# mingdeyu/DGP

Measured on AMD Instinct MI355X. Metric: SI iterations/sec (train) + predict pts/sec, 2-layer DGP n=2000 d=5, higher is better.
Workload: dtype f64; 1 GPU; configs[1]: 2-layer DGP, d=5 in / 1 out, n=2000, Matern-2.5, 5+1 GP nodes, train(ess_burn=10): one step = imputer.sample() + the M-step = one iteration of dgp.train (dgp.py:1364-1412); the same rate over a train(N=100) call is in `sustained`

## Files before the change

### dgp_amd/_lib.py

```python
import ctypes as C
import os

_HERE = os.path.dirname(os.path.abspath(__file__))
LIB_PATH = os.environ.get('DGPAMD_LIB') or os.path.join(_HERE, 'libdgp_amd.so')

OK, NOT_PD, BAD_ARG, HIP_ERROR = 0, 1, 2, 3
SEXP, MATERN25 = 0, 1
MAXD, MAXB = 64, 64
KIND = {'sexp': SEXP, 'matern2.5': MATERN25}

if not os.path.exists(LIB_PATH):
    raise ImportError(
        'dgp_amd: %s not found -- build it with `python -c "import __graft_entry__ as g; g.build()"` '
        '(or `make -C dgp_amd/csrc`).  dgp_amd has no CPU fallback.' % LIB_PATH)

lib = C.CDLL(LIB_PATH)

_p = C.c_void_p
_i = C.c_int
_l = C.c_int64
_d = C.c_double
_z = C.c_size_t

class Node(C.Structure):
# ... 21 lines not shown
    'dgpamd_gemv': (_i, [_p, _l, _l, _p, _l, _p, _p]),
    'dgpamd_fetch': (_i, [_p, _p, _p, _z]),
    'dgpamd_fetch2': (_i, [_p, _p, _z, _p, _z, _p]),
    'dgpamd_set_reduce_hook': (_i, [_p, _p, _p]),
    'dgpamd_post': (_i, [_p, _p, _z, _i]),
    'dgpamd_collect': (_i, [_p, _i, _p, _z]),
    'dgpamd_set_graphs': (_i, [_p, _i]),
    'dgpamd_tuning_get': (_i, [_p, C.c_char_p, _p]),
    'dgpamd_set_linkgp_direct': (_i, [_p, _i]),
    'dgpamd_set_potrf_mode': (_i, [_p, _i]),
    'dgpamd_debug_trace': (_i, [_p, _p]),
    'dgpamd_debug_tasklog': (_i, [_p, _p, C.c_longlong]),
    'dgpamd_debug_mega_table': (_i, [_p, _l, _i, _i, _p, _l]),
    'dgpamd_prof_enable': (_i, [_p, _i]),
    'dgpamd_prof_event_overhead_us': (_i, [_p, C.POINTER(_d)]),
    'dgpamd_prof_collect': (_i, [_p, C.POINTER(_l), C.POINTER(_d), C.POINTER(_d)]),
    'dgpamd_kmatrix': (_i, [_p, _i, _l, _p, _l, _l, _p, _i, _p, _i, _p, _i, _d, _p, _p, _l, _l, _i, _p, _l, _l, _i, _i]),
    'dgpamd_potrf_workspace': (_z, [_l, _i]),
    'dgpamd_potrf': (_i, [_p, _l, _p, _l, _i, _p, _p, _p]),
    'dgpamd_aug_quad': (_i, [_p, _l, _p, _l, _i, _i, _p]),
    'dgpamd_loglik_finish': (_i, [_p, _l, _p, _l, _i, _p, _d, _p]),
    'dgpamd_loglik': (_i, [_p, _i, _l, _p, _l, _l, _p, _i, _p, _i, _p, _i, _d, _p, _d, _p, _p, _l, _i, _p, _p, _p]),
    'dgpamd_trmv_lower': (_i, [_p, _l, _p, _l, _p, _p, _p, _i]),
    'dgpamd_lik_workspace': (_z, [_i]),
    'dgpamd_lik_loglik': (_i, [_p, _p, _l, _i, _p, _l, _i, _p, _p]),
    'dgpamd_ess_propose': (_i, [_p, _l, _i, _p, _p, _p, _i, _p]),
    'dgpamd_potri': (_i, [_p, _l, _p, _p, _i, _p]),
    'dgpamd_potri_batched': (_i, [_p, _l, _p, _p, _l, _i, _i, _p]),
    'dgpamd_grad_workspace': (_z, [_l, _i]),
    'dgpamd_grad_reduce': (_i, [_p, _i, _l, _p, _l, _p, _i, _p, _i, _p, _i, _d, _p, _i, _p, _p, _p]),
    'dgpamd_ess_update': (_i, [_p, _l, _i, _p, _p, _p, _d, _d, _p, _p, _i, _i, _i, _p, _p, _p, _p, _p, _p]),
    'dgpamd_ess_queue_scratch': (_z, []),
    'dgpamd_ess_queue': (_i, [_p, _l, _i, _p, _p, _i, _p, _p, _i, _p, _p, _p, _i, _i, _i, _i, _i, _p, _p, _p, _p, _p]),
    'dgpamd_ess_queue_vwork': (_z, [_l, _i, _i]),
    'dgpamd_ess_queue_note_info': (_i, [_p, _p, _p, _i]),
    'dgpamd_llik_batch': (_i, [_p, _l, _i, _p, _p, _p, _p, _l, _p, _p, _p, _p, _l]),
    'dgpamd_llik_batch_launch': (_i, [_p, _l, _i, _p, _p, _p, _p, _l, _p, _p, _p, _l]),
    'dgpamd_llik_batch_wait': (_i, [_p, _p]),
    'dgpamd_potrf_inv': (_i, [_p, _l, _p, _p, _p, _l, _i, _p, _p, _p]),
    'dgpamd_gp_workspace': (_z, [_l, _l]),
    'dgpamd_gp_predict': (_i, [_p, _i, _l, _l, _i, _p, _p, _p, _i, _p, _l, _p, _i, _d, _d, _p, _p, _p]),
    'dgpamd_joint_workspace': (_z, [_l, _l, _i, _i]),
    'dgpamd_joint_cov': (_i, [_p, _i, _l, _l, _i, _i, _i, _p, _l, _p, _i, _p, _l, _p, _l, _l, _p, _l, _p, _i, _d, _d, _p, _l,
                              _p, _p]),
    'dgpamd_mvn_paths': (_i, [_p, _l, _i, _i, _i, _p, _l, _p, _l, _p, _l, _p, _l]),
    'dgpamd_linkgp_workspace': (_z, [_l, _l, _i]),
# ... 55 lines not shown
```

### dgp_amd/csrc/chol.hip

```cpp
#include "common.hpp"
#include "tile.hpp"
#include "diagfac.hpp"

__device__ __forceinline__ void diag_logdet(DiagShared &sh, int ncol, int k, int b, int bad, double *logdet, int32_t *info) {
    const int tid = threadIdx.x;
    if (tid < 64) {
        const double pv = sh.piv[tid];
        double v = (tid < ncol && pv > 0.0) ? log(pv) : 0.0;
#pragma unroll
        for (int off = 32; off > 0; off >>= 1) v += __shfl_down(v, off, 64);
        if (tid == 0) {
            const double ld0 = k == 0 ? 0.0 : __hip_atomic_load(logdet + b, __ATOMIC_RELAXED, __HIP_MEMORY_SCOPE_AGENT);
            __hip_atomic_store(logdet + b, ld0 + v, __ATOMIC_RELAXED, __HIP_MEMORY_SCOPE_AGENT);
            int inf = k == 0 ? 0 : __hip_atomic_load(info + b, __ATOMIC_RELAXED, __HIP_MEMORY_SCOPE_AGENT);
            if (bad && inf == 0) inf = k * 64 + bad;
            __hip_atomic_store(info + b, inf, __ATOMIC_RELAXED, __HIP_MEMORY_SCOPE_AGENT);
        }
    }
}

enum { G_TRTRI1 = 2, G_TRTRI2 = 3, G_LAUUM = 4 };

struct GemmArgs {
    double *A;
// ... 1145 lines not shown
        int q = t / r, q2 = t % r;
        quad[(int64_t)b * r * r + t] = -A[(int64_t)b * stride_a + (n + q) * ld + n + q2];
    }
}

struct TrmvArgs {
    const double *L;
    int64_t ld, stride_a, n;
    const double *z;
    double *out;
    double sscale[DGPAMD_MAXB];
};
__global__ __launch_bounds__(256) void trmv_lower_kernel(TrmvArgs a) {
    const int b = blockIdx.y, wave = threadIdx.x >> 6, lane = threadIdx.x & 63;
    const int64_t i = (int64_t)blockIdx.x * 4 + wave;
    if (i >= a.n) return;
    const double *row = a.L + (int64_t)b * a.stride_a + i * a.ld;
    const double *z = a.z + (int64_t)b * a.n;
    double s = 0.0;
    for (int64_t j = lane; j <= i; j += 64) s = fma(row[j], z[j], s);
#pragma unroll
    for (int off = 32; off > 0; off >>= 1) s += __shfl_down(s, off, 64);
    if (lane == 0) a.out[(int64_t)b * a.n + i] = a.sscale[b] * s;
}

size_t potrf_ws_doubles(int64_t n, int batch) {
    int64_t nbk = padded_dim(n) / 64;
    return (size_t)batch * nbk * 4096 + 2 * DGPAMD_MAXB;
}

static size_t mega_sync_bytes(int64_t nbk, int batch);
static size_t mega_sync_offset(int64_t n, int batch) {
    const size_t b = potrf_ws_doubles(n, batch) * sizeof(double) + 3 * DGPAMD_MAXB * sizeof(int32_t);
    return (b + 127) / 128 * 128;
}
static size_t mega_piv_offset(int64_t n, int batch) {
    return mega_sync_offset(n, batch) + mega_sync_bytes(padded_dim(n) / 64, batch);
}
extern "C" size_t dgpamd_potrf_workspace(int64_t n, int batch) {
    return mega_piv_offset(n, batch) + (size_t)batch * padded_dim(n) * sizeof(double);
}

struct TaskTable {
    int4 *dev = nullptr;
    std::vector<int> offset, count, nhead, npanel;
    std::vector<double> tile_ops;
// ... 482 lines not shown

extern "C" int dgpamd_gemv(dgpamd_ctx *ctx, int64_t rows, int64_t cols, const double *A, int64_t ld, const double *x,
                           double *out) {
    if (!ctx) return DGPAMD_BAD_ARG;
    if (rows <= 0 || cols <= 0 || !A || !x || !out || ld < cols) BAD_ARG(ctx, "bad arguments");
    hipLaunchKernelGGL(gemv_kernel, dim3((unsigned)((rows + 3) / 4)), dim3(256), 0, ctx->stream, A, ld, rows, cols, x, out);
    LAUNCH_CHECK(ctx);
    return DGPAMD_OK;
}

extern "C" int dgpamd_trmv_lower(dgpamd_ctx *ctx, int64_t n, const double *L, int64_t stride_a, const double *scale_h,
                                 const double *z, double *out, int batch) {
    if (!ctx) return DGPAMD_BAD_ARG;
    if (n <= 0 || !L || !z || !out || !scale_h) BAD_ARG(ctx, "null pointer or n <= 0");
    if (batch <= 0 || batch > DGPAMD_MAXB) BAD_ARG(ctx, "need 1 <= batch <= DGPAMD_MAXB");
    TrmvArgs a;
    a.L = L; a.ld = padded_dim(n); a.stride_a = stride_a; a.n = n; a.z = z; a.out = out;
    for (int b = 0; b < batch; ++b) a.sscale[b] = sqrt(scale_h[b]);
    hipLaunchKernelGGL(trmv_lower_kernel, dim3((unsigned)((n + 3) / 4), batch), dim3(256), 0, ctx->stream, a);
    LAUNCH_CHECK(ctx);
    return DGPAMD_OK;
}

static int potri_launches(dgpamd_ctx *ctx, int64_t n, double *A, double *Ainv, int64_t stride_a, int r, int batch,
                          void *work);

extern "C" int dgpamd_potri_batched(dgpamd_ctx *ctx, int64_t n, double *A, double *Ainv, int64_t stride_a, int r,
                                    int batch, void *work) {
    if (!ctx) return DGPAMD_BAD_ARG;
    if (n <= 0 || !A || !Ainv || !work || r < 0) BAD_ARG(ctx, "null pointer or n <= 0");
    if (batch <= 0 || batch > DGPAMD_MAXB) BAD_ARG(ctx, "need 1 <= batch <= DGPAMD_MAXB");
    const int64_t Np = padded_dim(n);
    if (n + r > Np) BAD_ARG(ctx, "too many right-hand sides");
    if (batch > 1 && stride_a < Np * Np) BAD_ARG(ctx, "stride_a < Np*Np");
    const std::array<uint64_t, 10> key = {2, (uint64_t)n, (uint64_t)r, (uint64_t)A, (uint64_t)Ainv, (uint64_t)work,
                                          (uint64_t)batch, (uint64_t)stride_a, 0, 0};
    return graph_run(ctx, key, [&]() { return potri_launches(ctx, n, A, Ainv, stride_a, r, batch, work); });
}

extern "C" int dgpamd_potri(dgpamd_ctx *ctx, int64_t n, double *A, double *Ainv, int r, void *work) {
    return dgpamd_potri_batched(ctx, n, A, Ainv, 0, r, 1, work);
}

static int potri_launches(dgpamd_ctx *ctx, int64_t n, double *A, double *Ainv, int64_t stride_a, int r, int batch,
                          void *work) {
    const int64_t Np = padded_dim(n);
// ... 22 lines not shown
```

### dgp_amd/csrc/train.hip

```cpp
#include "common.hpp"
#include "wave.hpp"

#include <math.h>

struct ProposeArgs {
    const double *F, *NU;
    double *FP;
    int64_t count;
    double th[DGPAMD_MAXB];
};
__global__ __launch_bounds__(256) void ess_propose_kernel(ProposeArgs a) {
    const int b = blockIdx.y;
    const double c = cos(a.th[b]), s = sin(a.th[b]);
    for (int64_t i = (int64_t)blockIdx.x * 256 + threadIdx.x; i < a.count; i += (int64_t)gridDim.x * 256)
        a.FP[(int64_t)b * a.count + i] = a.F[i] * c + a.NU[i] * s;
}

extern "C" int dgpamd_ess_propose(dgpamd_ctx *ctx, int64_t n, int M, const double *F, const double *NU,
                                  const double *theta_h, int batch, double *FP) {
    if (!ctx) return DGPAMD_BAD_ARG;
    if (n <= 0 || M <= 0 || !F || !NU || !theta_h || !FP) BAD_ARG(ctx, "null pointer or empty block");
    if (batch <= 0 || batch > DGPAMD_MAXB) BAD_ARG(ctx, "need 1 <= batch <= DGPAMD_MAXB");
    ProposeArgs a;
    a.F = F; a.NU = NU; a.FP = FP; a.count = n * M;
// ... 636 lines not shown
            }
            if (llh[b] > log_y) {
                used += b;
                proposals += b + 1;
                theta = th[b]; lo = blo[b]; hi = bhi[b];
                HIP_TRY(ctx, hipMemcpyAsync(F, FP + (int64_t)b * n * M, sizeof(double) * n * M, hipMemcpyDeviceToDevice,
                                            ctx->stream));
                return finish(0, llh[b], 0);
            }
        }
        used += nb - 1;
        proposals += nb;
        theta = th[nb - 1]; lo = blo[nb - 1]; hi = bhi[nb - 1];
        pending = true;
    }
}

enum { ES_THETA = 0, ES_LO, ES_HI, ES_PENDING, ES_CURSOR, ES_STATUS, ES_INFO, ES_LL, ES_LOGY, ES_PROPOSALS, ES_BATCHES,
       ES_UPDATES, ES_NWORDS = DGPAMD_ESS_STATE };
struct EssScratch {
    double th[DGPAMD_MAXB], lo[DGPAMD_MAXB], hi[DGPAMD_MAXB], cs[DGPAMD_MAXB], sn[DGPAMD_MAXB], ll[DGPAMD_MAXB], logdet[DGPAMD_MAXB];
    int32_t info[DGPAMD_MAXB], infomax[DGPAMD_MAXB];
    int32_t nb, done, acc, halt;
    double likpart[DGPAMD_MAXB * 32];
};
#define ESS_TWO_PI 6.283185307179586

__device__ void ess_prepare(double *st, const double *u, int nuni, int B, EssScratch *sc);
__global__ void ess_begin_kernel(double *st, const double *u, const double *logu, int nuni, EssScratch *sc, int upd, int B, int resume) {
    if (threadIdx.x) return;
    if (resume && upd == 0) {
        sc->done = 0;
        sc->halt = 0;
        ess_prepare(st, u, nuni, B, sc);
        return;
    }
    if (upd > 0 && !sc->done && st[ES_STATUS] == 0.0) st[ES_STATUS] = 3.0;
    sc->acc = -1;
    sc->nb = 0;
    if (st[ES_STATUS] != 0.0) { sc->done = 1; sc->halt = 1; return; }
    int cur = (int)st[ES_CURSOR];
    if (cur + 2 > nuni) { st[ES_STATUS] = 4.0; sc->done = 1; sc->halt = 1; return; }
    st[ES_LOGY] = st[ES_LL] + logu[cur];
    const double theta = ESS_TWO_PI * u[cur + 1];
    st[ES_THETA] = theta; st[ES_LO] = theta - ESS_TWO_PI; st[ES_HI] = theta; st[ES_PENDING] = 0.0;
    st[ES_CURSOR] = cur + 2;
    sc->done = 0;
    sc->halt = 0;
    ess_prepare(st, u, nuni, B, sc);
}
__device__ void ess_prepare(double *st, const double *u, int nuni, int B, EssScratch *sc) {
    sc->acc = -1;
    sc->nb = 0;
    if (sc->done) return;
    int cur = (int)st[ES_CURSOR];
    double theta = st[ES_THETA], lo = st[ES_LO], hi = st[ES_HI];
    if (st[ES_PENDING] != 0.0) {
        if (cur >= nuni) { st[ES_STATUS] = 1.0; sc->done = 1; return; }
        if (theta < 0.0) lo = theta; else hi = theta;
        theta = __dadd_rn(lo, __dmul_rn(hi - lo, u[cur++]));
        st[ES_THETA] = theta; st[ES_LO] = lo; st[ES_HI] = hi; st[ES_PENDING] = 0.0; st[ES_CURSOR] = cur;
    }
    int nb = 1;
    sc->th[0] = theta; sc->lo[0] = lo; sc->hi[0] = hi;
    while (nb < B && cur + nb - 1 < nuni) {
        if (theta < 0.0) lo = theta; else hi = theta;
        theta = __dadd_rn(lo, __dmul_rn(hi - lo, u[cur + nb - 1]));
        sc->th[nb] = theta; sc->lo[nb] = lo; sc->hi[nb] = hi;
        ++nb;
    }
    for (int b = nb; b < B; ++b) sc->th[b] = sc->th[nb - 1];
    for (int b = 0; b < B; ++b) { sc->cs[b] = cos(sc->th[b]); sc->sn[b] = sin(sc->th[b]); }
    sc->nb = nb;
}
__global__ void ess_prepare_kernel(double *st, const double *u, int nuni, int B, EssScratch *sc) {
    if (threadIdx.x) return;
    ess_prepare(st, u, nuni, B, sc);
}
__global__ __launch_bounds__(256) void ess_propose_dev_kernel(const double *F, const double *NU, double *FP, int64_t count,
                                                              const EssScratch *sc) {
    if (sc->done) return;
    const int b = blockIdx.y;
    const double c = sc->cs[b], s = sc->sn[b];
    for (int64_t i = (int64_t)blockIdx.x * 256 + threadIdx.x; i < count; i += (int64_t)gridDim.x * 256)
        FP[(int64_t)b * count + i] = F[i] * c + NU[i] * s;
}
__device__ void ess_decide(double *st, EssScratch *sc);
__global__ void ess_node_ll_kernel(const double *A, int64_t ld, int64_t stride_a, int64_t n, double scale, int B, int first,
                                   EssScratch *sc, const double *ld_ws, const int32_t *info_ws, const int32_t *status, double *st) {
    const int b = threadIdx.x;
    if (sc->done) return;
    if (b < B) {
        const double logdet = ld_ws ? __hip_atomic_load(ld_ws + b, __ATOMIC_RELAXED, __HIP_MEMORY_SCOPE_AGENT) : sc->logdet[b];
        const int32_t info = ld_ws ? ((status && __hip_atomic_load(status, __ATOMIC_RELAXED, __HIP_MEMORY_SCOPE_AGENT))
                                          ? -1 : __hip_atomic_load(info_ws + b, __ATOMIC_RELAXED, __HIP_MEMORY_SCOPE_AGENT))
                                   : sc->info[b];
        const double quad = -A[(int64_t)b * stride_a + n * ld + n];
        const double ll = -0.5 * ((double)n * log(scale) + logdet + quad / scale);
        sc->ll[b] = (first ? 0.0 : sc->ll[b]) + ll;
        sc->infomax[b] = first ? info : (sc->infomax[b] ? sc->infomax[b] : info);
    }
    if (st) {
        __threadfence_block();
        __syncthreads();
        if (b == 0) ess_decide(st, sc);
    }
}
__device__ void ess_decide(double *st, EssScratch *sc) {
    if (sc->done) return;
    const int nb = sc->nb;
    int cur = (int)st[ES_CURSOR];
    st[ES_BATCHES] += 1.0;
    for (int b = 0; b < nb; ++b) {
        if (sc->infomax[b] != 0) {
            st[ES_STATUS] = 2.0; st[ES_INFO] = sc->infomax[b]; st[ES_PROPOSALS] += b + 1; sc->done = 1;
            return;
        }
        if (sc->ll[b] > st[ES_LOGY]) {
            st[ES_CURSOR] = cur + b; st[ES_PROPOSALS] += b + 1;
            st[ES_THETA] = sc->th[b]; st[ES_LO] = sc->lo[b]; st[ES_HI] = sc->hi[b]; st[ES_PENDING] = 0.0;
            st[ES_LL] = sc->ll[b]; st[ES_UPDATES] += 1.0;
            sc->acc = b; sc->done = 1;
            return;
        }
    }
    st[ES_CURSOR] = cur + nb - 1; st[ES_PROPOSALS] += nb;
    st[ES_THETA] = sc->th[nb - 1]; st[ES_LO] = sc->lo[nb - 1]; st[ES_HI] = sc->hi[nb - 1]; st[ES_PENDING] = 1.0;
}
__global__ __launch_bounds__(256) void ess_accept_kernel(double *F, const double *FP, int64_t count, const EssScratch *sc) {
    const int acc = sc->acc;
    if (acc < 0) return;
    for (int64_t i = (int64_t)blockIdx.x * 256 + threadIdx.x; i < count; i += (int64_t)gridDim.x * 256)
        F[i] = FP[(int64_t)acc * count + i];
}
__global__ void ess_end_kernel(double *st, EssScratch *sc) {
    if (threadIdx.x) return;
    if (!sc->done && st[ES_STATUS] == 0.0) st[ES_STATUS] = 3.0;
    sc->acc = -1;
}
__global__ void ess_set_ll_kernel(double *st, const EssScratch *sc) {
    if (threadIdx.x) return;
    if (st[ES_STATUS] != 0.0) return;
    if (sc->infomax[0] != 0) { st[ES_STATUS] = 2.0; st[ES_INFO] = sc->infomax[0]; }
    st[ES_LL] = sc->ll[0];
}
__global__ void ess_note_info_kernel(double *st, const int32_t *info, int count) {
    if (threadIdx.x || st[ES_STATUS] != 0.0) return;
    for (int i = 0; i < count; ++i)
        if (info[i] != 0) { st[ES_STATUS] = 2.0; st[ES_INFO] = info[i]; return; }
}

struct VGatherArgs {
    const double *X;
    int64_t stride_x;
    int M, Dl, Dg;
    int colmap[DGPAMD_MAXD];
    const double *Xglob;
    const int64_t *ord;
    int64_t n;
    double *out;
    const int32_t *pred;
};
__global__ __launch_bounds__(256) void ess_vgather_kernel(VGatherArgs a) {
    if (a.pred && *a.pred) return;
    const int D = a.Dl + a.Dg, b = blockIdx.y;
    const int64_t total = a.n * D;
    for (int64_t e = (int64_t)blockIdx.x * 256 + threadIdx.x; e < total; e += (int64_t)gridDim.x * 256) {
        const int64_t i = e / D;
        const int d = (int)(e - i * D);
        const int64_t src = a.ord[i];
        a.out[(int64_t)b * total + e] = d < a.Dl ? a.X[(int64_t)b * a.stride_x + src * a.M + a.colmap[d]] : a.Xglob[src * a.Dg + (d - a.Dl)];
    }
}
__global__ void ess_vnode_ll_kernel(const double *o, double scale, int B, int first, EssScratch *sc, double *st) {
    const int b = threadIdx.x;
    if (sc->done) return;
    if (b < B) {
        const double ll = -0.5 * (o[2 * b + 1] + o[2 * b] / scale);
        sc->ll[b] = (first ? 0.0 : sc->ll[b]) + ll;
        if (first) sc->infomax[b] = 0;
    }
    if (st) {
        __threadfence_block();
        __syncthreads();
        if (b == 0) ess_decide(st, sc);
    }
}

#define LIK_CHUNKS 32
struct LikArgs {
    const double *X;
    int64_t stride_x;
    int M, kind, ncol, classes;
    int cols[DGPAMD_MAXD];
    const int64_t *rep;
    const double *y;
    int64_t nobs;
    double par;
    double *part;
    const int32_t *pred;
};
__device__ __forceinline__ double lik_logaddexp(double a, double b) {
    if (a == b) return a + 0.6931471805599453;
    const double d = a - b;
    if (d > 0.0) return a + log1p(exp(-d));
    if (d <= 0.0) return b + log1p(exp(d));
    return a + b;
}
// ... 85 lines not shown
    const int b = blockIdx.y, ch = blockIdx.x, tid = threadIdx.x;
    const int64_t per = (a.nobs + LIK_CHUNKS - 1) / LIK_CHUNKS, lo = ch * per, hi = lo + per < a.nobs ? lo + per : a.nobs;
    const double *Xb = a.X + (int64_t)b * a.stride_x;
    double acc = 0.0;
    for (int64_t i = lo + tid; i < hi; i += 256) {
        const int64_t row = a.rep ? a.rep[i] : i;
        acc += lik_point(a, Xb + row * a.M, a.y[i]);
    }
    red[tid] = acc;
    __syncthreads();
    for (int w = 128; w > 0; w >>= 1) {
        if (tid < w) red[tid] += red[tid + w];
        __syncthreads();
    }
    if (tid == 0) a.part[b * LIK_CHUNKS + ch] = red[0];
}
__global__ void lik_sum_kernel(const double *part, int B, double *out) {
    const int b = threadIdx.x;
    if (b >= B) return;
    double s = 0.0;
    for (int c = 0; c < LIK_CHUNKS; ++c) s += part[b * LIK_CHUNKS + c];
    out[b] = s;
}
__global__ void ess_liknode_ll_kernel(const double *part, int B, int first, EssScratch *sc, double *st) {
    const int b = threadIdx.x;
    if (sc->done) return;
    if (b < B) {
        double s = 0.0;
        for (int c = 0; c < LIK_CHUNKS; ++c) s += part[b * LIK_CHUNKS + c];
        sc->ll[b] = (first ? 0.0 : sc->ll[b]) + s;
        if (first) sc->infomax[b] = 0;
    }
    if (st) {
        __threadfence_block();
        __syncthreads();
        if (b == 0) ess_decide(st, sc);
    }
}
static int lik_launch(dgpamd_ctx *ctx, const dgpamd_node &nd, int64_t n, int M, const double *X, int64_t stride_x, int B, double *part) {
    if (nd.lik_kind < DGPAMD_LIK_POISSON || nd.lik_kind > DGPAMD_LIK_SOFTMAX) BAD_ARG(ctx, "unknown likelihood");
    if (!nd.y || nd.lik_nobs <= 0 || !nd.colmap || nd.Dl <= 0 || nd.Dl > DGPAMD_MAXD) BAD_ARG(ctx, "incomplete likelihood node");
    static const int need[] = {0, 1, 2, 2, 3, 1, 1, 0, 0};
    if (need[nd.lik_kind] && nd.Dl != need[nd.lik_kind]) BAD_ARG(ctx, "wrong number of latent columns for this likelihood");
    if (nd.lik_kind >= DGPAMD_LIK_ROBUSTMAX && (nd.lik_classes != nd.Dl || nd.Dl < 2)) BAD_ARG(ctx, "one latent column per class");
    if (!nd.lik_rep && nd.lik_nobs != n) BAD_ARG(ctx, "observations and latent rows differ without a replicate map");
    LikArgs a;
    a.X = X; a.stride_x = stride_x; a.M = M; a.kind = nd.lik_kind; a.ncol = nd.Dl; a.classes = nd.lik_classes;
    for (int d = 0; d < nd.Dl; ++d) {
        a.cols[d] = ((const int32_t *)nd.colmap)[d];
        if (a.cols[d] < 0 || a.cols[d] >= M) BAD_ARG(ctx, "latent column out of range");
    }
    a.rep = nd.lik_rep; a.y = nd.y; a.nobs = nd.lik_nobs; a.par = nd.lik_par; a.part = part; a.pred = ctx->pred;
    hipLaunchKernelGGL(lik_partial_kernel, dim3(LIK_CHUNKS, B), dim3(256), 0, ctx->stream, a);
    return DGPAMD_OK;
}
extern "C" int dgpamd_lik_loglik(dgpamd_ctx *ctx, const dgpamd_node *node, int64_t n, int M, const double *X, int64_t stride_x, int batch,
                                 double *work, double *out) {
    if (!ctx) return DGPAMD_BAD_ARG;
    if (!node || !X || !work || !out || n <= 0 || M <= 0 || batch <= 0 || batch > DGPAMD_MAXB) BAD_ARG(ctx, "bad arguments");
    int rc = lik_launch(ctx, *node, n, M, X, stride_x, batch, work);
    if (rc) return rc;
    hipLaunchKernelGGL(lik_sum_kernel, dim3(1), dim3(DGPAMD_MAXB), 0, ctx->stream, (const double *)work, batch, out);
    LAUNCH_CHECK(ctx);
    return DGPAMD_OK;
}
extern "C" size_t dgpamd_lik_workspace(int batch) { return (size_t)batch * LIK_CHUNKS * sizeof(double); }

extern "C" size_t dgpamd_ess_queue_scratch(void) { return (sizeof(EssScratch) + 15) / 16 * 16; }
extern "C" size_t dgpamd_ess_queue_vwork(int64_t n, int D, int batch) {
    return ((size_t)batch * n * (D + 2) + 2 * (size_t)batch + 2) * sizeof(double);
}

static int ess_queue_logliks(dgpamd_ctx *ctx, int64_t n, int M, const double *X, int64_t stride_x, int B, const dgpamd_node *nodes,
                             const double *scales_h, int nnodes, double *A, void *work, EssScratch *sc, double *st_decide, void *vwork,
                             int vbatch) {
    const int64_t Np = padded_dim(n);
    double *ws = (double *)work;
    for (int k = 0; k < nnodes; ++k) {
        const dgpamd_node &nd = nodes[k];
        if (nd.lik_kind) {
            int rc = lik_launch(ctx, nd, n, M, X, stride_x, B, sc->likpart);
            if (rc) return rc;
            hipLaunchKernelGGL(ess_liknode_ll_kernel, dim3(1), dim3(DGPAMD_MAXB), 0, ctx->stream, (const double *)sc->likpart, B,
                               k == 0 ? 1 : 0, sc, k == nnodes - 1 ? st_decide : nullptr);
            continue;
        }
        if (!(scales_h[k] > 0.0)) BAD_ARG(ctx, "scale must be positive");
        if (nd.vecch_nn) {
            const int D = nd.Dl + nd.Dg;
            if (!vwork || !nd.vecch_ord || !nd.vecch_nd || !nd.vecch_y || nd.vecch_m < 0) BAD_ARG(ctx, "incomplete Vecchia node");
            if (D <= 0 || D > DGPAMD_MAXD) BAD_ARG(ctx, "need 1 <= Dl+Dg <= DGPAMD_MAXD");
            double *Xall = (double *)vwork, *partial = Xall + (size_t)vbatch * n * D, *osum = partial + (size_t)vbatch * n * 2;
            VGatherArgs ga;
            ga.X = X; ga.stride_x = stride_x; ga.M = M; ga.Dl = nd.Dl; ga.Dg = nd.Dg;
            for (int d = 0; d < nd.Dl; ++d) ga.colmap[d] = nd.colmap ? ((const int32_t *)nd.colmap)[d] : d;
            ga.Xglob = nd.Xglob; ga.ord = nd.vecch_ord; ga.n = n; ga.out = Xall; ga.pred = ctx->pred;
            int64_t gb = (n * D + 255) / 256;
            if (gb > 2048) gb = 2048;
            hipLaunchKernelGGL(ess_vgather_kernel, dim3((unsigned)gb, B), dim3(256), 0, ctx->stream, ga);
            const bool part = nd.vecch_rows > 0;
            if (part && (nd.vecch_row0 < 0 || nd.vecch_row0 + nd.vecch_rows > n)) BAD_ARG(ctx, "row block outside the neighbour array");
            if (part && !ctx->reduce_hook) BAD_ARG(ctx, "a row block needs a reduce hook (dgpamd_set_reduce_hook)");
            const int64_t rows = part ? nd.vecch_rows : n;
            int rc = vecchia_llik_batch_into(ctx, nd.kind, rows, D, nd.vecch_m, Xall, n * (int64_t)D, B, nd.vecch_y,
                                             nd.vecch_nn + (part ? nd.vecch_row0 * (nd.vecch_m + 1) : 0), nd.length, nd.nlen, nd.nugget,
                                             nd.vecch_nd, partial, osum);
            if (rc) return rc;
            if (part) {
                const hipStream_t was = ctx->stream;
                if (ctx->reduce_hook(ctx->reduce_user, osum, 2 * B) != 0 || ctx->stream != was) BAD_ARG(ctx, "the reduce hook failed");
            }
            hipLaunchKernelGGL(ess_vnode_ll_kernel, dim3(1), dim3(DGPAMD_MAXB), 0, ctx->stream, (const double *)osum, scales_h[k], B,
                               k == 0 ? 1 : 0, sc, k == nnodes - 1 ? st_decide : nullptr);
            continue;
        }
        if (!A || !work) BAD_ARG(ctx, "dense nodes upstairs need A and work");
        KmatArgs a;
        int rc = build_kmat_args(ctx, a, nd.kind, n, X, M, stride_x, (const int32_t *)nd.colmap, nd.Dl, nd.Xglob, nd.Dg, nd.length,
                                 nd.nlen, nd.nugget, nd.W, A, Np, Np * Np, 0, nd.y, n, 0, 1, B);
        if (rc) return rc;
        potrf_sync_area(ctx, n, B, false, ws, &a.zero_ptr, &a.zero_words);
        rc = launch_kmatrix(ctx, a, B);
        if (rc) return rc;
        PotrfPost post;
        rc = run_potrf(ctx, n, A, Np * Np, B, sc->logdet, sc->info, ws, nullptr, nullptr, &post, a.zero_ptr != nullptr);
        if (rc) return rc;
        hipLaunchKernelGGL(ess_node_ll_kernel, dim3(1), dim3(DGPAMD_MAXB), 0, ctx->stream, (const double *)A, Np, Np * Np, n,
                           scales_h[k], B, k == 0 ? 1 : 0, sc, post.pending ? post.ld_ws : nullptr,
                           post.pending ? post.info_ws : nullptr, post.pending ? post.status : nullptr,
                           k == nnodes - 1 ? st_decide : nullptr);
    }
    LAUNCH_CHECK(ctx);
    return DGPAMD_OK;
}

extern "C" int dgpamd_ess_queue(dgpamd_ctx *ctx, int64_t n, int M, double *F, const double *NU, int nupd, const dgpamd_node *nodes,
                                const double *scales_h, int nnodes, double *state, const double *uniforms, const double *log_uniforms,
                                int nuni, int batch_first, int batch_next, int max_batches, int compute_ll0, double *FP, double *A,
                                void *work, void *scratch, void *vwork) {
    if (!ctx) return DGPAMD_BAD_ARG;
    if (n <= 0 || M <= 0 || nupd <= 0 || nnodes <= 0 || !F || !NU || !nodes || !scales_h || !state || !FP || !scratch)
        BAD_ARG(ctx, "null pointer or empty block");
    if (nuni < 0 || (nuni > 0 && (!uniforms || !log_uniforms))) BAD_ARG(ctx, "bad uniform stream");
    if (batch_first <= 0 || batch_first > DGPAMD_MAXB) BAD_ARG(ctx, "need 1 <= batch_first <= DGPAMD_MAXB");
    if (batch_next <= 0 || batch_next > batch_first) batch_next = batch_first;
    if (max_batches < 1) max_batches = 1;
    EssScratch *sc = reinterpret_cast<EssScratch *>(scratch);
    const int64_t count = n * (int64_t)M;
    int64_t blocks = (count + 255) / 256;
    if (blocks > 1024) blocks = 1024;
    int rc;
    HIP_TRY(ctx, hipMemsetAsync(sc, 0, sizeof(EssScratch), ctx->stream));
    const int resume = compute_ll0 == 2 ? 1 : 0;
    if (compute_ll0 == 1) {
        rc = ess_queue_logliks(ctx, n, M, F, 0, 1, nodes, scales_h, nnodes, A, work, sc, nullptr, vwork, batch_first);
        if (rc) return rc;
        hipLaunchKernelGGL(ess_set_ll_kernel, dim3(1), dim3(64), 0, ctx->stream, state, (const EssScratch *)sc);
    }
    for (int u = 0; u < nupd; ++u) {
        const double *NUu = NU + (int64_t)u * count;
        hipLaunchKernelGGL(ess_begin_kernel, dim3(1), dim3(64), 0, ctx->stream, state, uniforms, log_uniforms, nuni, sc, u, batch_first, resume);
        for (int j = 0; j < max_batches; ++j) {
            const int B = j == 0 ? batch_first : batch_next;
            if (j > 0) hipLaunchKernelGGL(ess_prepare_kernel, dim3(1), dim3(64), 0, ctx->stream, state, uniforms, nuni, B, sc);
            hipLaunchKernelGGL(ess_propose_dev_kernel, dim3((unsigned)blocks, B), dim3(256), 0, ctx->stream, (const double *)F, NUu, FP,
                               count, (const EssScratch *)sc);
            ctx->pred = &sc->done;
            rc = ess_queue_logliks(ctx, n, M, FP, count, B, nodes, scales_h, nnodes, A, work, sc, state, vwork, batch_first);
            ctx->pred = nullptr;
            if (rc) return rc;
            hipLaunchKernelGGL(ess_accept_kernel, dim3((unsigned)blocks), dim3(256), 0, ctx->stream, F, (const double *)FP, count,
                               (const EssScratch *)sc);
        }
        if (u == nupd - 1) hipLaunchKernelGGL(ess_end_kernel, dim3(1), dim3(64), 0, ctx->stream, state, sc);
    }
    LAUNCH_CHECK(ctx);
    return DGPAMD_OK;
}

extern "C" int dgpamd_ess_queue_note_info(dgpamd_ctx *ctx, double *state, const int32_t *info, int count) {
    if (!ctx) return DGPAMD_BAD_ARG;
    if (!state || !info || count <= 0) BAD_ARG(ctx, "bad arguments");
    hipLaunchKernelGGL(ess_note_info_kernel, dim3(1), dim3(64), 0, ctx->stream, state, info, count);
    LAUNCH_CHECK(ctx);
    return DGPAMD_OK;
}
```

### dgp_amd/imputation.py

```python
import os
import numpy as np
from numpy.linalg import LinAlgError
from .ops import raise_not_pd
from . import dist as ddist
import torch

from .ops import default_engine
from .kernel_class import TrackedInputs, bind_private, peek

TWO_PI = 2.0 * np.pi
_NO_UPLOAD_AHEAD = bool(__import__('os').environ.get('DGPAMD_NO_UPLOAD_AHEAD'))


class DrawStream:

    def __init__(self, seed=None, z=None, u=None):
        ss = seed if isinstance(seed, np.random.SeedSequence) else np.random.SeedSequence(seed)
        a, b = ss.spawn(2)
        self._gz, self._gu = np.random.default_rng(a), np.random.default_rng(b)
        self._z = None if z is None else [np.asarray(v, dtype=float) for v in z]
        self._ubuf = [] if u is None else [float(v) for v in u]
        self._injected_u = u is not None
        self._zbuf, self._zpos, self._thread = None, 0, None

# ... 658 lines not shown
        layer = self.all_layer[0]
        if not self.block or any(nd.type != 'gp' for nd in layer):
            return None
        all_vecch = all(nd.vecch for nd in layer)
        if any(nd.vecch for nd in layer) and not all_vecch:
            return None
        if any(nd.type == 'likelihood' and getattr(nd, 'exact_post_idx', None) is not None for nd in self.all_layer[1]):
            return None
        if self.draws._z is not None and len(self.all_layer) > 2:
            return None
        e = self.engine
        n, M = self.F[0].shape
        if M > 64:
            return None
        if all_vecch:
            Zd = self._normals_ahead(sweeps, M, n)
            xs = self._vecchia_draws(0, list(range(M)), Zd.permute(1, 0, 2).contiguous())
            if prefetch:
                self.draws.prefetch(sweeps * M * n, engine=e)
            return xs.permute(1, 2, 0).contiguous()
        buf = self._layer_factors(0, list(range(M)))
        Zd = self._normals_ahead(sweeps, M, n)
        scales = [float(nd.scale[0]) for nd in layer]
        out = e.empty(sweeps, M, n)
        for s_ in range(sweeps):
            e.trmv_lower(n, buf, scales, Zd[s_], batch=M, out=out[s_])
        if prefetch:
            self.draws.prefetch(sweeps * M * n, engine=e)
        return out.transpose(1, 2).contiguous()

    def _prior_draw(self, l, cols=None):
        e = self.engine
        layer = self.all_layer[l]
        n, M = self.F[l].shape
        Np = e.padded_dim(n)
        nu = e.zeros(n, M)
        cols = list(range(M)) if cols is None else list(cols)
        dense = [k for k in cols if not layer[k].vecch]
        Z = {k: self.draws.normal(n) for k in cols}
        if dense:
            buf = self._layer_factors(l, dense)
            Zd = e.tensor(np.stack([Z[k] for k in dense]))
            scales = [float(layer[k].scale[0]) for k in dense]
            for c0 in range(0, len(dense), 64):
                nb = min(64, len(dense) - c0)
                out = e.trmv_lower(n, buf[c0:c0 + nb], scales[c0:c0 + nb], Zd[c0:c0 + nb], batch=nb)
                nu[:, torch.as_tensor(dense[c0:c0 + nb], device=nu.device)] = out.t()
        vec = [k for k in cols if layer[k].vecch]
        if vec:
# ... 346 lines not shown
```

### dgp_amd/ops.py

```python
import ctypes as C

import numpy as np
import torch

import os

from . import _lib
from ._lib import lib, KIND

_NO_PINNED_UPLOAD = os.environ.get('DGPAMD_PINNED_UPLOAD') == '0'
_POISON_ALL = os.environ.get('DGPAMD_POISON_LDS') == '2'
_POISON_HBM = os.environ.get('DGPAMD_POISON_HBM') == '1'


class DgpAmdError(RuntimeError):
    pass


class HandoffError(DgpAmdError):
    """The one-launch factorisation gave up waiting for another workgroup (its workgroups were not co-resident: a device
    shared with another process, a debugger, a time-sliced partition).  Not a numerical failure; the per-block-step
    factorisation (Engine.set_potrf_mode(0)) has no such waits -- dgp.train retries the iteration once through it."""


# ... 226 lines not shown
        Np = self.padded_dim(n)
        if A is None:
            A = self.workspace(('loglikA', n, batch), batch * Np * Np * 8)
        work = self.potrf_workspace(n, batch)
        if ll is None:
            ll = self.empty(batch)
        if info is None:
            info = self.empty(batch, dtype=torch.int32)
        stride_loc = n * ldloc if Xloc.dim() == 3 else 0
        self._chk(self._enter() or lib.dgpamd_loglik(self.h, KIND[kind], n, _dp(Xloc), ldloc, stride_loc, cmp_, Dl, _dp(Xglob), Dg,
                                    _hp(length), len(length), float(nugget), _dp(W), float(scale), _dp(y), _dp(A),
                                    Np * Np, batch, _dp(ll), _dp(info), _dp(work)))
        return ll, info

    def trmv_lower(self, n, L, scale, z, batch=1, out=None, shared=False):
        Np = self.padded_dim(n)
        sc = _f64(scale)
        if len(sc) == 1 and batch > 1:
            sc = np.repeat(sc, batch)
        if out is None:
            out = self.empty(batch, n)
        self._chk(self._enter() or lib.dgpamd_trmv_lower(self.h, n, _dp(L), 0 if shared else Np * Np, _hp(sc), _dp(z), _dp(out),
                                                          batch))
        return out

    def ess_propose(self, F, NU, thetas, out=None):
        n, M = F.shape
        th = _f64(thetas)
        B = len(th)
        if out is None:
            out = self.empty(B, n, M)
        self._chk(self._enter() or lib.dgpamd_ess_propose(self.h, n, M, _dp(F), _dp(NU), _hp(th), B, _dp(out)))
        return out

    def potri(self, n, A, Ainv, r, work, batch=1):
        Np = self.padded_dim(n)
        self._chk(self._enter() or lib.dgpamd_potri_batched(self.h, n, _dp(A), _dp(Ainv), Np * Np if batch > 1 else 0, r, batch, _dp(work)))
        return Ainv

    def grad_reduce(self, kind, Xloc, colmap, Xglob, length, nugget, nugget_est, Ainv, W=None):
        n, ldloc = Xloc.shape[-2], Xloc.shape[-1]
        Dl = ldloc if colmap is None else len(colmap)
        Dg = 0 if Xglob is None else Xglob.shape[1]
        cm, cmp_ = self._colmap(colmap, Dl)
        length = _f64(length)
        P = (1 if len(length) == 1 else Dl + Dg) + (1 if nugget_est else 0)
# ... 871 lines not shown
```

### include/dgp_amd.h

```cpp
#ifndef DGP_AMD_H
#define DGP_AMD_H

#include <stddef.h>
#include <stdint.h>

#ifdef __cplusplus
extern "C" {
#endif

#define DGPAMD_OK 0
#define DGPAMD_NOT_PD 1
#define DGPAMD_BAD_ARG 2
#define DGPAMD_HIP_ERROR 3

#define DGPAMD_SEXP 0
#define DGPAMD_MATERN25 1

#define DGPAMD_MAXD 64
#define DGPAMD_MAXB 64

typedef struct dgpamd_ctx dgpamd_ctx;

int dgpamd_create(int device, void *stream, dgpamd_ctx **out);
int dgpamd_destroy(dgpamd_ctx *ctx);
// ... 30 lines not shown
                   int batch);

size_t dgpamd_potrf_workspace(int64_t n, int batch);
int dgpamd_potrf(dgpamd_ctx *ctx, int64_t n, double *A, int64_t stride_a, int batch,
                 double *logdet, int32_t *info, void *work);
int dgpamd_set_potrf_mode(dgpamd_ctx *ctx, int mode);

int dgpamd_aug_quad(dgpamd_ctx *ctx, int64_t n, const double *A, int64_t stride_a, int batch, int r, double *quad);

int dgpamd_loglik_finish(dgpamd_ctx *ctx, int64_t n, const double *A, int64_t stride_a, int batch, const double *logdet,
                         double scale, double *ll);

int dgpamd_gemv(dgpamd_ctx *ctx, int64_t rows, int64_t cols, const double *A, int64_t ld, const double *x, double *out);

int dgpamd_loglik(dgpamd_ctx *ctx, int kind, int64_t n,
                  const double *Xloc, int64_t ldloc, int64_t stride_loc, const int32_t *colmap_h, int Dl,
                  const double *Xglob, int Dg,
                  const double *length_h, int nlen, double nugget, const double *W, double scale,
                  const double *y, double *A, int64_t stride_a, int batch,
                  double *ll, int32_t *info, void *work);

int dgpamd_trmv_lower(dgpamd_ctx *ctx, int64_t n, const double *L, int64_t stride_a, const double *scale_h,
                      const double *z, double *out, int batch);

int dgpamd_ess_propose(dgpamd_ctx *ctx, int64_t n, int M, const double *F, const double *NU,
                       const double *theta_h, int batch, double *FP);

int dgpamd_potri(dgpamd_ctx *ctx, int64_t n, double *A, double *Ainv, int r, void *work);
int dgpamd_potrf_inv(dgpamd_ctx *ctx, int64_t n, double *A, double *T, double *S, int64_t stride_a, int batch,
                     double *logdet, int32_t *info, void *work);

int dgpamd_potri_batched(dgpamd_ctx *ctx, int64_t n, double *A, double *Ainv, int64_t stride_a, int r, int batch,
                         void *work);

typedef struct {
    int kind;
    int Dl, Dg, nlen;
    int nugget_est;
    int reserved;
    int64_t ldloc;
    const double *Xloc;
    const int32_t *colmap;
    const double *Xglob;
    const double *length;
    double nugget;
    const double *W;
// ... 225 lines not shown
```

Baseline: 31.68 SI it/s.

## Fuse ESS accept/prepare/propose kernels and batch multi-RHS triangular matvecs

The ESS queue drops the separate begin, prepare, propose and accept kernels per batch. A single turn kernel now applies the previous accepted proposal and builds the new proposals, and the next-batch preparation is folded into the last log-likelihood decide kernel through a new accp field. Separately, the prior-draw triangular matvec over many sweeps becomes one multi-RHS kernel that reads each row of L once for up to four right-hand sides. Both aim to cut launch count and repeated reads of L, at the cost of more complex device-side control state.

```diff
diff --git a/dgp_amd/_lib.py b/dgp_amd/_lib.py
--- a/dgp_amd/_lib.py
+++ b/dgp_amd/_lib.py
@@ -67,6 +67,7 @@
     'dgpamd_loglik_finish': (_i, [_p, _l, _p, _l, _i, _p, _d, _p]),
     'dgpamd_loglik': (_i, [_p, _i, _l, _p, _l, _l, _p, _i, _p, _i, _p, _i, _d, _p, _d, _p, _p, _l, _i, _p, _p, _p]),
     'dgpamd_trmv_lower': (_i, [_p, _l, _p, _l, _p, _p, _p, _i]),
+    'dgpamd_trmv_lower_multi': (_i, [_p, _l, _p, _l, _p, _p, _l, _p, _l, _i, _i]),
     'dgpamd_lik_workspace': (_z, [_i]),
     'dgpamd_lik_loglik': (_i, [_p, _p, _l, _i, _p, _l, _i, _p, _p]),
     'dgpamd_ess_propose': (_i, [_p, _l, _i, _p, _p, _p, _i, _p]),
diff --git a/dgp_amd/csrc/chol.hip b/dgp_amd/csrc/chol.hip
--- a/dgp_amd/csrc/chol.hip
+++ b/dgp_amd/csrc/chol.hip
@@ -1191,6 +1191,57 @@
 #pragma unroll
     for (int off = 32; off > 0; off >>= 1) s += __shfl_down(s, off, 64);
     if (lane == 0) a.out[(int64_t)b * a.n + i] = a.sscale[b] * s;
+}
+
+#define TRMV_RHS 4
+#define TRMV_STEPS 4
+template <int NR>
+__device__ __forceinline__ void trmv_row_chunk(const double *row, const double *z, int64_t stride_z, double *out, int64_t stride_out,
+                                               int64_t i, int lane, double sscale) {
+    double s[NR];
+#pragma unroll
+    for (int q = 0; q < NR; ++q) s[q] = 0.0;
+    int64_t j = lane;
+    for (; j + 64 * (TRMV_STEPS - 1) <= i; j += 64 * TRMV_STEPS) {
+        double l[TRMV_STEPS], zz[TRMV_STEPS][NR];
+#pragma unroll
+        for (int k = 0; k < TRMV_STEPS; ++k) {
+            l[k] = row[j + 64 * k];
+#pragma unroll
+            for (int q = 0; q < NR; ++q) zz[k][q] = z[(int64_t)q * stride_z + j + 64 * k];
+        }
+#pragma unroll
+        for (int k = 0; k < TRMV_STEPS; ++k)
+#pragma unroll
+            for (int q = 0; q < NR; ++q) s[q] = fma(l[k], zz[k][q], s[q]);
+    }
+    for (; j <= i; j += 64) {
+        const double l = row[j];
+#pragma unroll
+        for (int q = 0; q < NR; ++q) s[q] = fma(l, z[(int64_t)q * stride_z + j], s[q]);
+    }
+#pragma unroll
+    for (int q = 0; q < NR; ++q) {
+#pragma unroll
+        for (int off = 32; off > 0; off >>= 1) s[q] += __shfl_down(s[q], off, 64);
+        if (lane == 0) out[(int64_t)q * stride_out] = sscale * s[q];
+    }
+}
+__global__ __launch_bounds__(256) void trmv_lower_multi_kernel(TrmvArgs a, int nrhs, int64_t stride_z, int64_t stride_out) {
+    const int b = blockIdx.y, wave = threadIdx.x >> 6, lane = threadIdx.x & 63;
+    const int64_t i = (int64_t)blockIdx.x * 4 + wave;
+    if (i >= a.n) return;
+    const double *row = a.L + (int64_t)b * a.stride_a + i * a.ld;
+    for (int r0 = 0; r0 < nrhs; r0 += TRMV_RHS) {
+        const double *z = a.z + (int64_t)r0 * stride_z + (int64_t)b * a.n;
+        double *out = a.out + (int64_t)r0 * stride_out + (int64_t)b * a.n + i;
+        switch (nrhs - r0) {
+        case 1: trmv_row_chunk<1>(row, z, stride_z, out, stride_out, i, lane, a.sscale[b]); break;
+        case 2: trmv_row_chunk<2>(row, z, stride_z, out, stride_out, i, lane, a.sscale[b]); break;
+        case 3: trmv_row_chunk<3>(row, z, stride_z, out, stride_out, i, lane, a.sscale[b]); break;
+        default: trmv_row_chunk<TRMV_RHS>(row, z, stride_z, out, stride_out, i, lane, a.sscale[b]); break;
+        }
+    }
 }
 
 size_t potrf_ws_doubles(int64_t n, int batch) {
@@ -1719,6 +1770,22 @@
     return DGPAMD_OK;
 }
 
+extern "C" int dgpamd_trmv_lower_multi(dgpamd_ctx *ctx, int64_t n, const double *L, int64_t stride_a, const double *scale_h,
+                                       const double *z, int64_t stride_z, double *out, int64_t stride_out, int batch, int nrhs) {
+    if (!ctx) return DGPAMD_BAD_ARG;
+    if (n <= 0 || !L || !z || !out || !scale_h) BAD_ARG(ctx, "null pointer or n <= 0");
+    if (batch <= 0 || batch > DGPAMD_MAXB) BAD_ARG(ctx, "need 1 <= batch <= DGPAMD_MAXB");
+    if (nrhs <= 0) BAD_ARG(ctx, "need nrhs >= 1");
+    if (nrhs > 1 && (stride_z < (int64_t)batch * n || stride_out < (int64_t)batch * n)) BAD_ARG(ctx, "stride < batch * n");
+    TrmvArgs a;
+    a.L = L; a.ld = padded_dim(n); a.stride_a = stride_a; a.n = n; a.z = z; a.out = out;
+    for (int b = 0; b < batch; ++b) a.sscale[b] = sqrt(scale_h[b]);
+    hipLaunchKernelGGL(trmv_lower_multi_kernel, dim3((unsigned)((n + 3) / 4), batch), dim3(256), 0, ctx->stream, a, nrhs, stride_z,
+                       stride_out);
+    LAUNCH_CHECK(ctx);
+    return DGPAMD_OK;
+}
+
 static int potri_launches(dgpamd_ctx *ctx, int64_t n, double *A, double *Ainv, int64_t stride_a, int r, int batch,
                           void *work);
 
diff --git a/dgp_amd/csrc/train.hip b/dgp_amd/csrc/train.hip
--- a/dgp_amd/csrc/train.hip
+++ b/dgp_amd/csrc/train.hip
@@ -682,13 +682,13 @@
     double th[DGPAMD_MAXB], lo[DGPAMD_MAXB], hi[DGPAMD_MAXB], cs[DGPAMD_MAXB], sn[DGPAMD_MAXB], ll[DGPAMD_MAXB], logdet[DGPAMD_MAXB];
     int32_t info[DGPAMD_MAXB], infomax[DGPAMD_MAXB];
     int32_t nb, done, acc, halt;
+    int32_t accp, pad_[3];
     double likpart[DGPAMD_MAXB * 32];
 };
 #define ESS_TWO_PI 6.283185307179586
 
 __device__ void ess_prepare(double *st, const double *u, int nuni, int B, EssScratch *sc);
-__global__ void ess_begin_kernel(double *st, const double *u, const double *logu, int nuni, EssScratch *sc, int upd, int B, int resume) {
-    if (threadIdx.x) return;
+__device__ void ess_begin(double *st, const double *u, const double *logu, int nuni, EssScratch *sc, int upd, int B, int resume) {
     if (resume && upd == 0) {
         sc->done = 0;
         sc->halt = 0;
@@ -709,6 +709,11 @@
     sc->halt = 0;
     ess_prepare(st, u, nuni, B, sc);
 }
+__global__ void ess_begin_kernel(double *st, const double *u, const double *logu, int nuni, EssScratch *sc, int upd, int B, int resume) {
+    if (threadIdx.x) return;
+    ess_begin(st, u, logu, nuni, sc, upd, B, resume);
+    sc->accp = -1;
+}
 __device__ void ess_prepare(double *st, const double *u, int nuni, int B, EssScratch *sc) {
     sc->acc = -1;
     sc->nb = 0;
@@ -733,24 +738,44 @@
     for (int b = 0; b < B; ++b) { sc->cs[b] = cos(sc->th[b]); sc->sn[b] = sin(sc->th[b]); }
     sc->nb = nb;
 }
-__global__ void ess_prepare_kernel(double *st, const double *u, int nuni, int B, EssScratch *sc) {
-    if (threadIdx.x) return;
-    ess_prepare(st, u, nuni, B, sc);
-}
-__global__ __launch_bounds__(256) void ess_propose_dev_kernel(const double *F, const double *NU, double *FP, int64_t count,
-                                                              const EssScratch *sc) {
-    if (sc->done) return;
-    const int b = blockIdx.y;
-    const double c = sc->cs[b], s = sc->sn[b];
-    for (int64_t i = (int64_t)blockIdx.x * 256 + threadIdx.x; i < count; i += (int64_t)gridDim.x * 256)
-        FP[(int64_t)b * count + i] = F[i] * c + NU[i] * s;
+struct EssNext {
+    int kind;
+    int B, upd, nuni;
+    const double *u, *logu;
+};
+__device__ void ess_next(double *st, EssScratch *sc, const EssNext &nx) {
+    const int acc = sc->acc;
+    if (nx.kind == 1) ess_prepare(st, nx.u, nx.nuni, nx.B, sc);
+    if (nx.kind == 2) ess_begin(st, nx.u, nx.logu, nx.nuni, sc, nx.upd, nx.B, 0);
+    sc->accp = acc;
+}
+__device__ __forceinline__ double ess_mix(double f, double c, double nu, double s) { return f * c + nu * s; }
+__global__ __launch_bounds__(256) void ess_turn_kernel(double *F, const double *NU, double *FP, int64_t count, int B,
+                                                       const EssScratch *sc) {
+    const int acc = sc->accp;
+    const bool open = !sc->done;
+    if (acc < 0 && !open) return;
+    for (int64_t i = (int64_t)blockIdx.x * 256 + threadIdx.x; i < count; i += (int64_t)gridDim.x * 256) {
+        double f;
+        if (acc >= 0) {
+            f = FP[(int64_t)acc * count + i];
+            F[i] = f;
+        } else
+            f = F[i];
+        if (open) {
+            const double nu = NU[i];
+            for (int b = 0; b < B; ++b) FP[(int64_t)b * count + i] = ess_mix(f, sc->cs[b], nu, sc->sn[b]);
+        }
+    }
 }
 __device__ void ess_decide(double *st, EssScratch *sc);
 __global__ void ess_node_ll_kernel(const double *A, int64_t ld, int64_t stride_a, int64_t n, double scale, int B, int first,
-                                   EssScratch *sc, const double *ld_ws, const int32_t *info_ws, const int32_t *status, double *st) {
+                                   EssScratch *sc, const double *ld_ws, const int32_t *info_ws, const int32_t *status, double *st,
+                                   EssNext nx) {
     const int b = threadIdx.x;
-    if (sc->done) return;
-    if (b < B) {
+    const bool open = !sc->done;
+    if (!open && !st) return;
+    if (open && b < B) {
         const double logdet = ld_ws ? __hip_atomic_load(ld_ws + b, __ATOMIC_RELAXED, __HIP_MEMORY_SCOPE_AGENT) : sc->logdet[b];
         const int32_t info = ld_ws ? ((status && __hip_atomic_load(status, __ATOMIC_RELAXED, __HIP_MEMORY_SCOPE_AGENT))
                                           ? -1 : __hip_atomic_load(info_ws + b, __ATOMIC_RELAXED, __HIP_MEMORY_SCOPE_AGENT))
@@ -763,7 +788,10 @@
     if (st) {
         __threadfence_block();
         __syncthreads();
-        if (b == 0) ess_decide(st, sc);
+        if (b == 0) {
+            if (open) ess_decide(st, sc);
+            ess_next(st, sc, nx);
+        }
     }
 }
 __device__ void ess_decide(double *st, EssScratch *sc) {
@@ -788,7 +816,7 @@
     st[ES_THETA] = sc->th[nb - 1]; st[ES_LO] = sc->lo[nb - 1]; st[ES_HI] = sc->hi[nb - 1]; st[ES_PENDING] = 1.0;
 }
 __global__ __launch_bounds__(256) void ess_accept_kernel(double *F, const double *FP, int64_t count, const EssScratch *sc) {
-    const int acc = sc->acc;
+    const int acc = sc->accp;
     if (acc < 0) return;
     for (int64_t i = (int64_t)blockIdx.x * 256 + threadIdx.x; i < count; i += (int64_t)gridDim.x * 256)
         F[i] = FP[(int64_t)acc * count + i];
@@ -832,10 +860,11 @@
         a.out[(int64_t)b * total + e] = d < a.Dl ? a.X[(int64_t)b * a.stride_x + src * a.M + a.colmap[d]] : a.Xglob[src * a.Dg + (d - a.Dl)];
     }
 }
-__global__ void ess_vnode_ll_kernel(const double *o, double scale, int B, int first, EssScratch *sc, double *st) {
+__global__ void ess_vnode_ll_kernel(const double *o, double scale, int B, int first, EssScratch *sc, double *st, EssNext nx) {
     const int b = threadIdx.x;
-    if (sc->done) return;
-    if (b < B) {
+    const bool open = !sc->done;
+    if (!open && !st) return;
+    if (open && b < B) {
         const double ll = -0.5 * (o[2 * b + 1] + o[2 * b] / scale);
         sc->ll[b] = (first ? 0.0 : sc->ll[b]) + ll;
         if (first) sc->infomax[b] = 0;
@@ -843,7 +872,10 @@
     if (st) {
         __threadfence_block();
         __syncthreads();
-        if (b == 0) ess_decide(st, sc);
+        if (b == 0) {
+            if (open) ess_decide(st, sc);
+            ess_next(st, sc, nx);
+        }
     }
 }
 
@@ -975,10 +1007,11 @@
     for (int c = 0; c < LIK_CHUNKS; ++c) s += part[b * LIK_CHUNKS + c];
     out[b] = s;
 }
-__global__ void ess_liknode_ll_kernel(const double *part, int B, int first, EssScratch *sc, double *st) {
+__global__ void ess_liknode_ll_kernel(const double *part, int B, int first, EssScratch *sc, double *st, EssNext nx) {
     const int b = threadIdx.x;
-    if (sc->done) return;
-    if (b < B) {
+    const bool open = !sc->done;
+    if (!open && !st) return;
+    if (open && b < B) {
         double s = 0.0;
         for (int c = 0; c < LIK_CHUNKS; ++c) s += part[b * LIK_CHUNKS + c];
         sc->ll[b] = (first ? 0.0 : sc->ll[b]) + s;
@@ -987,7 +1020,10 @@
     if (st) {
         __threadfence_block();
         __syncthreads();
-        if (b == 0) ess_decide(st, sc);
+        if (b == 0) {
+            if (open) ess_decide(st, sc);
+            ess_next(st, sc, nx);
+        }
     }
 }
 static int lik_launch(dgpamd_ctx *ctx, const dgpamd_node &nd, int64_t n, int M, const double *X, int64_t stride_x, int B, double *part) {
@@ -1026,8 +1062,11 @@
 
 static int ess_queue_logliks(dgpamd_ctx *ctx, int64_t n, int M, const double *X, int64_t stride_x, int B, const dgpamd_node *nodes,
                              const double *scales_h, int nnodes, double *A, void *work, EssScratch *sc, double *st_decide, void *vwork,
-                             int vbatch) {
+                             int vbatch, const EssNext *next = nullptr) {
     const int64_t Np = padded_dim(n);
+    EssNext nx;
+    memset(&nx, 0, sizeof(nx));
+    if (next && st_decide) nx = *next;
     double *ws = (double *)work;
     for (int k = 0; k < nnodes; ++k) {
         const dgpamd_node &nd = nodes[k];
@@ -1035,7 +1074,7 @@
             int rc = lik_launch(ctx, nd, n, M, X, stride_x, B, sc->likpart);
             if (rc) return rc;
             hipLaunchKernelGGL(ess_liknode_ll_kernel, dim3(1), dim3(DGPAMD_MAXB), 0, ctx->stream, (const double *)sc->likpart, B,
-                               k == 0 ? 1 : 0, sc, k == nnodes - 1 ? st_decide : nullptr);
+                               k == 0 ? 1 : 0, sc, k == nnodes - 1 ? st_decide : nullptr, nx);
             continue;
         }
         if (!(scales_h[k] > 0.0)) BAD_ARG(ctx, "scale must be positive");
@@ -1064,7 +1103,7 @@
                 if (ctx->reduce_hook(ctx->reduce_user, osum, 2 * B) != 0 || ctx->stream != was) BAD_ARG(ctx, "the reduce hook failed");
             }
             hipLaunchKernelGGL(ess_vnode_ll_kernel, dim3(1), dim3(DGPAMD_MAXB), 0, ctx->stream, (const double *)osum, scales_h[k], B,
-                               k == 0 ? 1 : 0, sc, k == nnodes - 1 ? st_decide : nullptr);
+                               k == 0 ? 1 : 0, sc, k == nnodes - 1 ? st_decide : nullptr, nx);
             continue;
         }
         if (!A || !work) BAD_ARG(ctx, "dense nodes upstairs need A and work");
@@ -1081,7 +1120,7 @@
         hipLaunchKernelGGL(ess_node_ll_kernel, dim3(1), dim3(DGPAMD_MAXB), 0, ctx->stream, (const double *)A, Np, Np * Np, n,
                            scales_h[k], B, k == 0 ? 1 : 0, sc, post.pending ? post.ld_ws : nullptr,
                            post.pending ? post.info_ws : nullptr, post.pending ? post.status : nullptr,
-                           k == nnodes - 1 ? st_decide : nullptr);
+                           k == nnodes - 1 ? st_decide : nullptr, nx);
     }
     LAUNCH_CHECK(ctx);
     return DGPAMD_OK;
@@ -1110,23 +1149,26 @@
         if (rc) return rc;
         hipLaunchKernelGGL(ess_set_ll_kernel, dim3(1), dim3(64), 0, ctx->stream, state, (const EssScratch *)sc);
     }
+    hipLaunchKernelGGL(ess_begin_kernel, dim3(1), dim3(64), 0, ctx->stream, state, uniforms, log_uniforms, nuni, sc, 0, batch_first, resume);
     for (int u = 0; u < nupd; ++u) {
         const double *NUu = NU + (int64_t)u * count;
-        hipLaunchKernelGGL(ess_begin_kernel, dim3(1), dim3(64), 0, ctx->stream, state, uniforms, log_uniforms, nuni, sc, u, batch_first, resume);
         for (int j = 0; j < max_batches; ++j) {
             const int B = j == 0 ? batch_first : batch_next;
-            if (j > 0) hipLaunchKernelGGL(ess_prepare_kernel, dim3(1), dim3(64), 0, ctx->stream, state, uniforms, nuni, B, sc);
-            hipLaunchKernelGGL(ess_propose_dev_kernel, dim3((unsigned)blocks, B), dim3(256), 0, ctx->stream, (const double *)F, NUu, FP,
-                               count, (const EssScratch *)sc);
+            hipLaunchKernelGGL(ess_turn_kernel, dim3((unsigned)blocks), dim3(256), 0, ctx->stream, F, NUu, FP, count, B,
+                               (const EssScratch *)sc);
+            EssNext nx;
+            memset(&nx, 0, sizeof(nx));
+            nx.u = uniforms; nx.logu = log_uniforms; nx.nuni = nuni;
+            if (j + 1 < max_batches) { nx.kind = 1; nx.B = batch_next; }
+            else if (u + 1 < nupd) { nx.kind = 2; nx.B = batch_first; nx.upd = u + 1; }
             ctx->pred = &sc->done;
-            rc = ess_queue_logliks(ctx, n, M, FP, count, B, nodes, scales_h, nnodes, A, work, sc, state, vwork, batch_first);
+            rc = ess_queue_logliks(ctx, n, M, FP, count, B, nodes, scales_h, nnodes, A, work, sc, state, vwork, batch_first, &nx);
             ctx->pred = nullptr;
             if (rc) return rc;
-            hipLaunchKernelGGL(ess_accept_kernel, dim3((unsigned)blocks), dim3(256), 0, ctx->stream, F, (const double *)FP, count,
-                               (const EssScratch *)sc);
-        }
-        if (u == nupd - 1) hipLaunchKernelGGL(ess_end_kernel, dim3(1), dim3(64), 0, ctx->stream, state, sc);
-    }
+        }
+    }
+    hipLaunchKernelGGL(ess_accept_kernel, dim3((unsigned)blocks), dim3(256), 0, ctx->stream, F, (const double *)FP, count, (const EssScratch *)sc);
+    hipLaunchKernelGGL(ess_end_kernel, dim3(1), dim3(64), 0, ctx->stream, state, sc);
     LAUNCH_CHECK(ctx);
     return DGPAMD_OK;
 }
diff --git a/dgp_amd/imputation.py b/dgp_amd/imputation.py
--- a/dgp_amd/imputation.py
+++ b/dgp_amd/imputation.py
@@ -704,9 +704,7 @@
         buf = self._layer_factors(0, list(range(M)))
         Zd = self._normals_ahead(sweeps, M, n)
         scales = [float(nd.scale[0]) for nd in layer]
-        out = e.empty(sweeps, M, n)
-        for s_ in range(sweeps):
-            e.trmv_lower(n, buf, scales, Zd[s_], batch=M, out=out[s_])
+        out = e.trmv_lower_multi(n, buf, scales, Zd, batch=M)
         if prefetch:
             self.draws.prefetch(sweeps * M * n, engine=e)
         return out.transpose(1, 2).contiguous()
diff --git a/dgp_amd/ops.py b/dgp_amd/ops.py
--- a/dgp_amd/ops.py
+++ b/dgp_amd/ops.py
@@ -272,6 +272,19 @@
             out = self.empty(batch, n)
         self._chk(self._enter() or lib.dgpamd_trmv_lower(self.h, n, _dp(L), 0 if shared else Np * Np, _hp(sc), _dp(z), _dp(out),
                                                           batch))
+        return out
+
+    def trmv_lower_multi(self, n, L, scale, z, batch=1, out=None, shared=False):
+        Np = self.padded_dim(n)
+        sc = _f64(scale)
+        if len(sc) == 1 and batch > 1:
+            sc = np.repeat(sc, batch)
+        nrhs = z.shape[0]
+        if out is None:
+            out = self.empty(nrhs, batch, n)
+        assert z.shape == (nrhs, batch, n) and out.shape == (nrhs, batch, n) and z.is_contiguous() and out.is_contiguous()
+        self._chk(self._enter() or lib.dgpamd_trmv_lower_multi(self.h, n, _dp(L), 0 if shared else Np * Np, _hp(sc), _dp(z), batch * n,
+                                                                _dp(out), batch * n, batch, nrhs))
         return out
 
     def ess_propose(self, F, NU, thetas, out=None):
diff --git a/include/dgp_amd.h b/include/dgp_amd.h
--- a/include/dgp_amd.h
+++ b/include/dgp_amd.h
@@ -76,6 +76,8 @@
 
 int dgpamd_trmv_lower(dgpamd_ctx *ctx, int64_t n, const double *L, int64_t stride_a, const double *scale_h,
                       const double *z, double *out, int batch);
+int dgpamd_trmv_lower_multi(dgpamd_ctx *ctx, int64_t n, const double *L, int64_t stride_a, const double *scale_h,
+                            const double *z, int64_t stride_z, double *out, int64_t stride_out, int batch, int nrhs);
 
 int dgpamd_ess_propose(dgpamd_ctx *ctx, int64_t n, int M, const double *F, const double *NU,
                        const double *theta_h, int batch, double *FP);
```

Measured after the change: 31.97 SI it/s (median of 3 runs). Within noise of the previous version (+0.9%).
